# hamidthri/navbot_ppo

Measured on AMD Instinct MI355X. Metric: env_steps_per_sec, higher is better.
Workload: dtype f32; 1 GPU; BASELINE configs[1]: 4096 envs/GPU, stage_1 (32 segments), 10 beams, PPO mlp64x2, rollout=512, 50 full-batch epochs, episode cap 500; n_envs_total=4096, n_envs_per_gpu=4096, rollout_len=512, epochs=50, policy=mlp64x2, parallelism=env-shard dp1, update_arith=bf16x3, rollout=persistent kernel (navsim_rollout_mlp64)

## Files before the change

### navbot_ppo_amd/csrc/ppo_mlp64_x3s.h

```cpp
#pragma once

namespace x3s {

typedef unsigned u32x4 __attribute__((ext_vector_type(4)));
typedef unsigned u32x2 __attribute__((ext_vector_type(2)));
typedef short s16x4 __attribute__((ext_vector_type(4)));
typedef float v4f __attribute__((ext_vector_type(4)));

constexpr int SW = 4;
constexpr int kPieceB = 32 * 128;
constexpr int kImgB = 3 * kPieceB;

struct SmemS {
    uint16_t W2p[3][H][H];
    uint16_t W2Tp[3][H][H];
    uint16_t W1p[3][H][16];
    float b1[H], b2[H], w3[H], w4[H];
    unsigned char img[SW][2][kImgB];
};
static_assert(sizeof(SmemS) <= 160 * 1024, "LDS");
static_assert(offsetof(SmemS, img) % 128 == 0 && kImgB % 128 == 0, "image bases keep the low 7 address bits of a lane offset (the XOR swizzles)");
static_assert(sizeof(SmemS::img) >= 4 * ((Layout<16>::P_ACTOR + 6) & ~3) * sizeof(float), "reduction rows fit the images");
static_assert(sizeof(SmemS::img) / SW >= 96 * 64 * sizeof(float), "lane partials fit a wave's images");

#ifndef X3S_GUARD
#define X3S_GUARD ""
#endif
#define X3S_G "s_nop 0\n\t"
#define X3S_MFMA32_V_AV(acc, A, B) asm volatile(X3S_GUARD "v_mfma_f32_32x32x16_bf16 %0, %1, %2, %0" : "+v"(acc) : "a"(A), "v"(B))
#define X3S_MFMA32_V_AA(acc, A, B) asm volatile(X3S_GUARD "v_mfma_f32_32x32x16_bf16 %0, %1, %2, %0" : "+v"(acc) : "a"(A), "a"(B))
#define X3S_MFMA32G_V_AV(acc, A, B) asm volatile(X3S_G "v_mfma_f32_32x32x16_bf16 %0, %1, %2, %0" : "+v"(acc) : "a"(A), "v"(B))
#define X3S_MFMA32G_V_AA(acc, A, B) asm volatile(X3S_G "v_mfma_f32_32x32x16_bf16 %0, %1, %2, %0" : "+v"(acc) : "a"(A), "a"(B))
#define X3S_MFMA32_VZ_AV(acc, A, B) asm volatile(X3S_G "v_mfma_f32_32x32x16_bf16 %0, %1, %2, 0" : "=&v"(acc) : "a"(A), "v"(B))
#define X3S_MFMA32_VZ_AA(acc, A, B) asm volatile(X3S_G "v_mfma_f32_32x32x16_bf16 %0, %1, %2, 0" : "=&v"(acc) : "a"(A), "a"(B))
#define X3S_MFMA32_A_AV(acc, A, B) asm volatile(X3S_GUARD "v_mfma_f32_32x32x16_bf16 %0, %1, %2, %0" : "+a"(acc) : "a"(A), "v"(B))
#define X3S_MFMA32_AZ_AV(acc, A, B) asm volatile(X3S_G "v_mfma_f32_32x32x16_bf16 %0, %1, %2, 0" : "=&a"(acc) : "a"(A), "v"(B))
#define X3S_MFMA32_A_AA(acc, A, B) asm volatile(X3S_GUARD "v_mfma_f32_32x32x16_bf16 %0, %1, %2, %0" : "+a"(acc) : "a"(A), "a"(B))
#define X3S_MFMA16_A_AA(acc, A, B) asm volatile(X3S_GUARD "v_mfma_f32_16x16x32_bf16 %0, %1, %2, %0" : "+a"(acc) : "a"(A), "a"(B))
#define X3S_MFMA16G_A_AA(acc, A, B) asm volatile(X3S_G "v_mfma_f32_16x16x32_bf16 %0, %1, %2, %0" : "+a"(acc) : "a"(A), "a"(B))
#define X3S_MFMA16_A_AV(acc, A, B) asm volatile(X3S_GUARD "v_mfma_f32_16x16x32_bf16 %0, %1, %2, %0" : "+a"(acc) : "a"(A), "v"(B))

__device__ __forceinline__ void settle(f32x16& a, f32x16& b) { asm volatile("s_nop 7\n\ts_nop 3" : "+v"(a), "+v"(b)); }

__device__ __forceinline__ void split_a(unsigned& p0, float& ra, float& rb, const float a, const float b) {
    asm volatile("v_cvt_pk_bf16_f32 %0, %3, %4\n\t"
                 "v_lshlrev_b32 %1, 16, %0\n\t"
                 "v_and_b32 %2, 0xffff0000, %0\n\t"
                 "v_sub_f32 %1, %3, %1\n\t"
                 "v_sub_f32 %2, %4, %2"
                 : "=&v"(p0), "=&v"(ra), "=&v"(rb) : "v"(a), "v"(b));
}
__device__ __forceinline__ void split_b(unsigned& p1, unsigned& p2, const float ra, const float rb) {
    float t0, t1;
    asm volatile("v_cvt_pk_bf16_f32 %0, %4, %5\n\t"
                 "v_lshlrev_b32 %2, 16, %0\n\t"
                 "v_and_b32 %3, 0xffff0000, %0\n\t"
                 "v_sub_f32 %2, %4, %2\n\t"
                 "v_sub_f32 %3, %5, %3\n\t"
                 "v_cvt_pk_bf16_f32 %1, %2, %3"
                 : "=&v"(p1), "=&v"(p2), "=&v"(t0), "=&v"(t1) : "v"(ra), "v"(rb));
}
__device__ __forceinline__ void relu4(float (&h)[16], const f32x16& c, const int g) {
    float y0, y1, y2, y3;
    asm volatile("v_max_i32 %0, %4, 0\n\tv_max_i32 %1, %5, 0\n\tv_max_i32 %2, %6, 0\n\tv_max_i32 %3, %7, 0"
                 : "=&v"(y0), "=&v"(y1), "=&v"(y2), "=&v"(y3) : "v"(c[4 * g]), "v"(c[4 * g + 1]), "v"(c[4 * g + 2]), "v"(c[4 * g + 3]));
    h[4 * g] = y0; h[4 * g + 1] = y1; h[4 * g + 2] = y2; h[4 * g + 3] = y3;
}
template <bool ACTOR>
__device__ __forceinline__ void dh2_value(float& h, float& pw3, float& pw4, float& pb2, const float g3, const float g4, const float w3,
                                          const float w4) {
    float d;
    if constexpr (ACTOR)
        asm volatile("v_fmac_f32 %1, %0, %5\n\t"
                     "v_fmac_f32 %2, %0, %6\n\t"
                     "v_mul_f32 %4, %6, %8\n\t"
                     "v_fmac_f32 %4, %5, %7\n\t"
                     "v_cmp_lt_f32 vcc, 0, %0\n\t"
                     "v_cndmask_b32 %0, 0, %4, vcc\n\t"
                     "v_add_f32 %3, %3, %0"
                     : "+v"(h), "+v"(pw3), "+v"(pw4), "+v"(pb2), "=&v"(d) : "v"(g3), "v"(g4), "v"(w3), "v"(w4) : "vcc");
    else
        asm volatile("v_fmac_f32 %1, %0, %4\n\t"
                     "v_mul_f32 %3, %4, %5\n\t"
                     "v_cmp_lt_f32 vcc, 0, %0\n\t"
                     "v_cndmask_b32 %0, 0, %3, vcc\n\t"
                     "v_add_f32 %2, %2, %0"
                     : "+v"(h), "+v"(pw3), "+v"(pb2), "=&v"(d) : "v"(g3), "v"(w3) : "vcc");
}

__device__ __forceinline__ void mask4(float& y0, float& y1, float& y2, float& y3, const float x0, const float x1, const float x2,
                                      const float x3, const unsigned w0, const unsigned w1) {
    asm volatile("v_cmp_ne_u16 vcc, 0, %8\n\t"
                 "v_cndmask_b32 %0, 0, %4, vcc\n\t"
                 "v_cmp_lt_u32 vcc, 0xffff, %8\n\t"
                 "v_cndmask_b32 %1, 0, %5, vcc\n\t"
                 "v_cmp_ne_u16 vcc, 0, %9\n\t"
                 "v_cndmask_b32 %2, 0, %6, vcc\n\t"
                 "v_cmp_lt_u32 vcc, 0xffff, %9\n\t"
                 "v_cndmask_b32 %3, 0, %7, vcc"
                 : "=&v"(y0), "=&v"(y1), "=&v"(y2), "=&v"(y3) : "v"(x0), "v"(x1), "v"(x2), "v"(x3), "v"(w0), "v"(w1) : "vcc");
}

struct P3 {
    u32x4 p[3];
};

__device__ __forceinline__ int fswz(const int m) { return (m & 3) | ((((m >> 2) ^ (m >> 3)) & 1) << 2) | ((((m >> 1) ^ (m >> 3)) & 1) << 3); }

typedef __attribute__((address_space(3))) s16x4* lds_s16x4;
__device__ __forceinline__ u32x2 tr_read(const unsigned char* p) {
    const s16x4 v = __builtin_amdgcn_ds_read_tr16_b64_v4i16((lds_s16x4)p);
    u32x2 r;
    __builtin_memcpy(&r, &v, 8);
    return r;
}
__device__ __forceinline__ u32x4 cat(const u32x2 lo, const u32x2 hi) { return u32x4{lo.x, lo.y, hi.x, hi.y}; }

template <bool ACTOR>
__device__ __forceinline__ void pass_body(SmemS& sm, const float* __restrict__ params, const unsigned char* __restrict__ prep,
                                          const float* __restrict__ act, const float* __restrict__ logp_old,
                                          const float* __restrict__ rtg, const float* __restrict__ adv, long long M, float var,
                                          float clip, float inv_n, float* __restrict__ partial, float* __restrict__ stats_partial) {
    using L = Layout<16>;
    constexpr int OFF_W1 = L::OFF_W1, OFF_B1 = L::OFF_B1, OFF_W2 = L::OFF_W2, OFF_B2 = L::OFF_B2, OFF_W3 = L::OFF_W3, OFF_B3 = L::OFF_B3,
                  OFF_W4 = L::OFF_W4, OFF_B4 = L::OFF_B4;
    constexpr int P = ACTOR ? L::P_ACTOR : L::P_CRITIC;
    constexpr int NT = 64 * SW, kTileBytes = XPad<16>::kTileBytes, kRowsBytes = XPad<16>::kRowsBytes;
    const int tid = threadIdx.x, lane = tid & 63, wave = __builtin_amdgcn_readfirstlane(tid >> 6);
    const int l31 = lane & 31, lhi = lane >> 5, l15 = lane & 15, kk = lane >> 4;

    for (int k = tid; k < H * H / 2; k += NT) {
        const int r = (2 * k) / H, c = (2 * k) % H;
        uint32_t p0, p1, p2;
        bf16x3::split_pair(params[OFF_W2 + r * H + c], params[OFF_W2 + r * H + c + 1], p0, p1, p2);
        const uint32_t pc[3] = {p0, p1, p2};
#pragma unroll
        for (int i = 0; i < 3; ++i) {
            *reinterpret_cast<uint32_t*>(&sm.W2p[i][0][0] + wslot(r, kpos(c))) = pc[i];
            (&sm.W2Tp[i][0][0])[wslot(c, kpos(r))] = (uint16_t)(pc[i] & 0xffffu);
            (&sm.W2Tp[i][0][0])[wslot(c + 1, kpos(r))] = (uint16_t)(pc[i] >> 16);
        }
    }
    for (int k = tid; k < H * 16 / 2; k += NT) {
        const int r = (2 * k) / 16, c = (2 * k) % 16;
        uint32_t p0, p1, p2;
        bf16x3::split_pair(params[OFF_W1 + r * 16 + c], params[OFF_W1 + r * 16 + c + 1], p0, p1, p2);
        *reinterpret_cast<uint32_t*>(&sm.W1p[0][r][c]) = p0;
        *reinterpret_cast<uint32_t*>(&sm.W1p[1][r][c]) = p1;
        *reinterpret_cast<uint32_t*>(&sm.W1p[2][r][c]) = p2;
    }
    if (tid < H) {
        sm.b1[tid] = params[OFF_B1 + tid];
        sm.b2[tid] = params[OFF_B2 + tid];
        sm.w3[tid] = params[OFF_W3 + tid];
        sm.w4[tid] = ACTOR ? params[OFF_W4 + tid] : 0.f;
    }
    const float b3 = params[OFF_B3];
    const float b4 = ACTOR ? params[OFF_B4] : 0.f;
    __syncthreads();

    unsigned char* const smb = reinterpret_cast<unsigned char*>(&sm);
    const int img0 = (int)offsetof(SmemS, img) + wave * 2 * kImgB;
    constexpr int IMG_H = 0, IMG_D = kImgB;
    const int st_base = img0 + l31 * 128 + ((fswz(l31) ^ lhi) << 3);
    auto st_off = [&](const int t, const int j, const int b) { return st_base ^ ((8 * t + 4 * j + 2 * b) << 3); };
    const int g_row = 8 * lhi + (l15 >> 2), g_quad = 4 * ((lane >> 4) & 1) + (lane & 3);
    const int g_base0 = img0 + g_row * 128 + ((g_quad ^ fswz(g_row)) << 3), g_base1 = img0 + (g_row + 4) * 128 + ((g_quad ^ fswz(g_row + 4)) << 3);
    auto g_off = [&](const int t, const int s, const int rd) { return ((rd ? g_base1 : g_base0) ^ (t << 6)) + s * 2048; };
    const int h_row = 8 * kk + (l15 >> 2), h_quad = lane & 3;
    const int h_base0 = img0 + h_row * 128 + ((h_quad ^ fswz(h_row)) << 3), h_base1 = img0 + (h_row + 4) * 128 + ((h_quad ^ fswz(h_row + 4)) << 3);
    auto ldw = [&](const uint16_t* base, const int tt, const int s, const int i) {
        return *reinterpret_cast<const u32x4*>(base + i * H * H + wslot(32 * tt + l31, 16 * s + 8 * lhi));
    };
    const int vec_off = 4 * lhi;
    auto ldv = [&](const float* v, const int t, const int g) { return *reinterpret_cast<const v4f*>(v + 32 * t + 8 * g + vec_off); };

    f32x16 aW2[2][2];
    v4f aW1[4], aB1[4];
#pragma unroll
    for (int a = 0; a < 2; ++a)
#pragma unroll
        for (int b = 0; b < 2; ++b) aW2[a][b] = zero16();
#pragma unroll
    for (int u = 0; u < 4; ++u) aW1[u] = aB1[u] = v4f{0.f, 0.f, 0.f, 0.f};
    float pb2[2][16], pw3[2][16], pw4[2][16];
#pragma unroll
    for (int t = 0; t < 2; ++t)
#pragma unroll
        for (int r = 0; r < 16; ++r) pb2[t][r] = pw3[t][r] = pw4[t][r] = 0.f;
    float adb3 = 0.f, adb4 = 0.f, st0 = 0.f, st1 = 0.f, st2 = 0.f, st3 = 0.f;
    u32x4 ones = {0x3f803f80u, 0x3f803f80u, 0x3f803f80u, 0x3f803f80u};
    asm volatile("" : "+a"(ones));

    const long long n_tiles = (M + 31) / 32;
    const long long gw = (long long)blockIdx.x * SW + wave, stride = (long long)gridDim.x * SW;
    u32x4 xp[3], xbn[3];
    float pre_a0 = 0.f, pre_a1 = 0.f, pre_lp = 0.f, pre_t = 0.f;
    auto request_tile = [&](const long long next, const long long cur) {
        const unsigned char* r = prep + (size_t)next * kTileBytes + ((l31 * 3) * 16 + 8 * lhi) * 2;
        const unsigned char* c = prep + (size_t)cur * kTileBytes + kRowsBytes + (l15 * 32 + 8 * kk) * 2;
        asm volatile("global_load_dwordx4 %0, %3, off\n\tglobal_load_dwordx4 %1, %3, off offset:32\n\tglobal_load_dwordx4 %2, %3, off offset:64"
                     : "=a"(xp[0]), "=a"(xp[1]), "=a"(xp[2]) : "v"(r));
        asm volatile("global_load_dwordx4 %0, %3, off\n\tglobal_load_dwordx4 %1, %3, off offset:1024\n\tglobal_load_dwordx4 %2, %3, off offset:2048"
                     : "=a"(xbn[0]), "=a"(xbn[1]), "=a"(xbn[2]) : "v"(c));
        const long long m = next * 32 + l31;
        if (m < M) {
            if (ACTOR) {
                const float2 a = reinterpret_cast<const float2*>(act)[m];
                pre_a0 = a.x;
                pre_a1 = a.y;
                pre_lp = logp_old[m];
                pre_t = adv[m];
            } else {
                pre_t = rtg[m];
            }
        }
    };
    auto landed = [&]() {
        asm volatile("s_waitcnt vmcnt(0)" : "+a"(xp[0]), "+a"(xp[1]), "+a"(xp[2]), "+a"(xbn[0]), "+a"(xbn[1]), "+a"(xbn[2]));
    };
    static_assert(kTileBytes == 6144 && kRowsBytes == 3072, "offsets of the asm loads: pieces 32 bytes apart in a row, 1024 in the columns");

    struct G1Ops {
        P3 da[4];
    };
    auto g1_gather_pair = [&](G1Ops& o, const int q, const int hb0, const int hb1) {
        const int u = q / 3, i = q % 3;
        o.da[u].p[i] = cat(tr_read(smb + (hb0 ^ (u << 5)) + IMG_D + i * kPieceB), tr_read(smb + (hb1 ^ (u << 5)) + IMG_D + i * kPieceB));
    };
    auto g1_step = [&](const int k, const G1Ops& o, const u32x4 (&xb)[3], const bool guard = false) {
        const int t1 = k / 18, q = k % 18, u = 2 * t1 + (q & 1), e = q >> 1;
        constexpr int kind[9] = {0, 1, 0, 0, 1, 0, 0, 1, 0};
        constexpr int ai[9] = {2, 2, 1, 0, 1, 1, 0, 0, 0};
        constexpr int bi[9] = {0, 0, 1, 2, 0, 0, 1, 0, 0};
        if (guard) {
            if (kind[e]) { X3S_MFMA16G_A_AA(aB1[u], o.da[u].p[ai[e]], ones); }
            else { X3S_MFMA16G_A_AA(aW1[u], o.da[u].p[ai[e]], xb[bi[e]]); }
        } else {
            if (kind[e]) { X3S_MFMA16_A_AA(aB1[u], o.da[u].p[ai[e]], ones); }
            else { X3S_MFMA16_A_AA(aW1[u], o.da[u].p[ai[e]], xb[bi[e]]); }
        }
    };
    auto store_pieces = [&](const int img, const int t, const int j, const P3& q) {
#pragma unroll
        for (int i = 0; i < 3; ++i) {
            *reinterpret_cast<u32x2*>(smb + st_off(t, j, 0) + img + i * kPieceB) = u32x2{q.p[i].x, q.p[i].y};
            *reinterpret_cast<u32x2*>(smb + st_off(t, j, 1) + img + i * kPieceB) = u32x2{q.p[i].z, q.p[i].w};
        }
    };
    struct SplitState {
        float ra[4], rb[4];
    };
    auto split_block = [&](const float (&c)[16], const int j, const int b, P3& q, SplitState& ss) {
        const int pr = b >> 1;
        if ((b & 1) == 0) {
            unsigned p0;
            split_a(p0, ss.ra[pr], ss.rb[pr], c[8 * j + 2 * pr], c[8 * j + 2 * pr + 1]);
            q.p[0][pr] = p0;
        } else {
            unsigned p1, p2;
            split_b(p1, p2, ss.ra[pr], ss.rb[pr]);
            q.p[1][pr] = p1;
            q.p[2][pr] = p2;
        }
    };

    for (int k = lane; k < kImgB / 16; k += 64) reinterpret_cast<u32x4*>(smb + img0 + IMG_D)[k] = u32x4{0u, 0u, 0u, 0u};
    bool have_prev = false;
    if (gw < n_tiles) {
        request_tile(gw, gw);
        landed();
    }
    for (long long tile = gw; tile < n_tiles; tile += stride) {
        const bool valid = tile * 32 + l31 < M;
        const u32x4 xr[3] = {xp[0], xp[1], xp[2]}, xb[3] = {xbn[0], xbn[1], xbn[2]};
        const float cur_a0 = pre_a0, cur_a1 = pre_a1, cur_lp = pre_lp, cur_t = pre_t;

        f32x16 c1[2];
#pragma unroll
        for (int q = 0; q < 8; ++q) {
            const v4f b = ldv(sm.b1, q >> 2, q & 3);
            c1[q >> 2][4 * (q & 3)] = b.x; c1[q >> 2][4 * (q & 3) + 1] = b.y; c1[q >> 2][4 * (q & 3) + 2] = b.z; c1[q >> 2][4 * (q & 3) + 3] = b.w;
        }
        {
            u32x4 wa[2][3];
#pragma unroll
            for (int t = 0; t < 2; ++t)
#pragma unroll
                for (int i = 0; i < 3; ++i) wa[t][i] = *reinterpret_cast<const u32x4*>(&sm.W1p[i][32 * t + l31][8 * lhi]);
            X3S_MFMA32G_V_AA(c1[0], wa[0][2], xr[0]); X3S_MFMA32G_V_AA(c1[1], wa[1][2], xr[0]);
            X3S_MFMA32_V_AA(c1[0], wa[0][1], xr[1]);  X3S_MFMA32_V_AA(c1[1], wa[1][1], xr[1]);
            X3S_MFMA32_V_AA(c1[0], wa[0][0], xr[2]);  X3S_MFMA32_V_AA(c1[1], wa[1][0], xr[2]);
            X3S_MFMA32_V_AA(c1[0], wa[0][1], xr[0]);  X3S_MFMA32_V_AA(c1[1], wa[1][1], xr[0]);
            X3S_MFMA32_V_AA(c1[0], wa[0][0], xr[1]);  X3S_MFMA32_V_AA(c1[1], wa[1][0], xr[1]);
            X3S_MFMA32_V_AA(c1[0], wa[0][0], xr[0]);  X3S_MFMA32_V_AA(c1[1], wa[1][0], xr[0]);
        }
        request_tile(tile + stride < n_tiles ? tile + stride : tile, tile);
        u32x4 wn[2][3];
#pragma unroll
        for (int i = 0; i < 3; ++i) {
            wn[0][i] = ldw(&sm.W2p[0][0][0], 0, 0, i);
            wn[1][i] = ldw(&sm.W2p[0][0][0], 1, 0, i);
        }
        settle(c1[0], c1[1]);
        float h1[2][16];
#pragma unroll
        for (int q = 0; q < 8; ++q) relu4(h1[q >> 2], c1[q >> 2], q & 3);
        f32x16 c2[2];
#pragma unroll
        for (int q = 0; q < 8; ++q) {
            const v4f b = ldv(sm.b2, q >> 2, q & 3);
            c2[q >> 2][4 * (q & 3)] = b.x; c2[q >> 2][4 * (q & 3) + 1] = b.y; c2[q >> 2][4 * (q & 3) + 2] = b.z; c2[q >> 2][4 * (q & 3) + 3] = b.w;
        }

        G1Ops g1o;
        {
            P3 hb[4];
            u32x4 wk[4][2];
            SplitState ss;
#pragma unroll
            for (int b = 0; b < 8; ++b) split_block(h1[0], 0, b, hb[0], ss);
#pragma unroll
            for (int s = 0; s < 4; ++s) {
                u32x4 w[2][3];
#pragma unroll
                for (int i = 0; i < 3; ++i) { w[0][i] = wn[0][i]; w[1][i] = wn[1][i]; }
                auto filler = [&](const int slot) {
                    if (s < 3 && slot >= 1 && slot <= 8) split_block(h1[(s + 1) >> 1], (s + 1) & 1, slot - 1, hb[s + 1], ss);
                    if (s == 3 && slot < 8) wk[slot >> 1][slot & 1] = ldw(&sm.W2p[0][0][0], slot & 1, slot >> 1, 0);
                    if (s < 3 && (slot == 0 || slot == 4 || slot == 9)) {
                        const int i = slot == 0 ? 0 : slot == 4 ? 1 : 2;
                        wn[0][i] = ldw(&sm.W2p[0][0][0], 0, s + 1, i);
                        wn[1][i] = ldw(&sm.W2p[0][0][0], 1, s + 1, i);
                    }
                    if (slot == 9) store_pieces(IMG_H, s >> 1, s & 1, hb[s]);
                };
                if (s == 0) { X3S_MFMA32G_V_AV(c2[0], w[0][2], hb[s].p[0]); } else { X3S_MFMA32_V_AV(c2[0], w[0][2], hb[s].p[0]); }
                filler(0);
                if (s == 0) { X3S_MFMA32G_V_AV(c2[1], w[1][2], hb[s].p[0]); } else { X3S_MFMA32_V_AV(c2[1], w[1][2], hb[s].p[0]); }
                filler(1);
                X3S_MFMA32_V_AV(c2[0], w[0][1], hb[s].p[1]); filler(2);
                X3S_MFMA32_V_AV(c2[1], w[1][1], hb[s].p[1]); filler(3);
                X3S_MFMA32_V_AV(c2[0], w[0][0], hb[s].p[2]); filler(4);
                X3S_MFMA32_V_AV(c2[1], w[1][0], hb[s].p[2]); filler(5);
                X3S_MFMA32_V_AV(c2[0], w[0][1], hb[s].p[0]); filler(6);
                X3S_MFMA32_V_AV(c2[1], w[1][1], hb[s].p[0]); filler(7);
                X3S_MFMA32_V_AV(c2[0], w[0][0], hb[s].p[1]); filler(8);
                X3S_MFMA32_V_AV(c2[1], w[1][0], hb[s].p[1]); filler(9);
            }
            int hb0 = h_base0, hb1 = h_base1;
            asm volatile("" : "+v"(hb0), "+v"(hb1));
            int gq = 0;
#pragma unroll
            for (int s = 0; s < 4; ++s) {
                X3S_MFMA32_V_AV(c2[0], wk[s][0], hb[s].p[0]);
                g1_gather_pair(g1o, gq++, hb0, hb1); g1_gather_pair(g1o, gq++, hb0, hb1);
                X3S_MFMA32_V_AV(c2[1], wk[s][1], hb[s].p[0]);
                g1_gather_pair(g1o, gq++, hb0, hb1);
            }
        }
        settle(c2[0], c2[1]);

        int g1k = 0;
        float h2[2][16];
#pragma unroll
        for (int q = 0; q < 8; ++q) {
            relu4(h2[q >> 2], c2[q >> 2], q & 3);
            g1_step(g1k++, g1o, xb);
            g1_step(g1k++, g1o, xb);
        }
        float g3 = 0.f, g4 = 0.f;
        {
            float z3 = 0.f, z4 = 0.f;
#pragma unroll
            for (int t = 0; t < 2; ++t)
#pragma unroll
                for (int g = 0; g < 4; ++g) {
                    const v4f w = ldv(sm.w3, t, g);
                    z3 = fmaf(h2[t][4 * g], w.x, z3); z3 = fmaf(h2[t][4 * g + 1], w.y, z3);
                    z3 = fmaf(h2[t][4 * g + 2], w.z, z3); z3 = fmaf(h2[t][4 * g + 3], w.w, z3);
                    if (ACTOR) {
                        const v4f v = ldv(sm.w4, t, g);
                        z4 = fmaf(h2[t][4 * g], v.x, z4); z4 = fmaf(h2[t][4 * g + 1], v.y, z4);
                        z4 = fmaf(h2[t][4 * g + 2], v.z, z4); z4 = fmaf(h2[t][4 * g + 3], v.w, z4);
                    }
                }
            z3 += __shfl_xor(z3, 32, 64);
            if (ACTOR) z4 += __shfl_xor(z4, 32, 64);
            const float own = (lhi == 0) ? 1.f : 0.f;
            if (valid) {
                z3 += b3;
                z4 += b4;
#ifdef MLP64_DEBUG_Z
                if (lhi == 0) {
                    float* const dbg = partial + (size_t)200 * P;
                    dbg[tile * 32 + l31] = z3;
                    if (ACTOR) dbg[M + tile * 32 + l31] = z4;
                }
#endif
                if (ACTOR) {
                    const float mu0 = 1.0f / (1.0f + expf(-z3));
                    const float mu1 = tanhf(z4);
                    const float d0 = cur_a0 - mu0, d1 = cur_a1 - mu1;
                    const float lp = -0.5f * ((d0 * d0 + d1 * d1) / var) - 1.8378770664093453f - logf(var);
                    const float lr = lp - cur_lp;
                    const float ratio = expf(lr);
                    const float A = cur_t;
                    const float s1 = ratio * A;
                    const float rc = fminf(fmaxf(ratio, 1.0f - clip), 1.0f + clip);
                    const float s2 = rc * A;
                    st0 += own * -fminf(s1, s2);
                    st2 += own * ((ratio - 1.0f) - lr);
                    st3 += (fabsf(ratio - 1.0f) > clip) ? own : 0.f;
                    const bool inside = (ratio >= 1.0f - clip) && (ratio <= 1.0f + clip);
                    const float dL_dratio = (inside || s1 < s2) ? -A : 0.f;
                    const float dL_dlp = dL_dratio * ratio * inv_n;
                    g3 = dL_dlp * (d0 / var) * (mu0 * (1.0f - mu0));
                    g4 = dL_dlp * (d1 / var) * (1.0f - mu1 * mu1);
                } else {
                    const float e = z3 - cur_t;
                    st1 += own * (e * e);
                    g3 = 2.0f * e * inv_n;
                }
            }
            adb3 += own * g3;
            adb4 += own * g4;
#ifdef MLP64_DEBUG_Z
            if (valid && lhi == 0) {
                float* const dbg = partial + (size_t)200 * P;
                dbg[2 * M + tile * 32 + l31] = g3;
                if (ACTOR) dbg[3 * M + tile * 32 + l31] = g4;
            }
#endif
        }
        {
            v4f wn3 = ldv(sm.w3, 0, 0), wn4 = ACTOR ? ldv(sm.w4, 0, 0) : v4f{0.f, 0.f, 0.f, 0.f};
#pragma unroll
            for (int q = 0; q < 8; ++q) {
                const int t = q >> 2, g = q & 3;
                const v4f w = wn3, v = wn4;
                if (q < 7) {
                    wn3 = ldv(sm.w3, (q + 1) >> 2, (q + 1) & 3);
                    if (ACTOR) wn4 = ldv(sm.w4, (q + 1) >> 2, (q + 1) & 3);
                }
                const float wv3[4] = {w.x, w.y, w.z, w.w}, wv4[4] = {v.x, v.y, v.z, v.w};
#pragma unroll
                for (int j = 0; j < 4; ++j) {
                    const int r = 4 * g + j;
                    dh2_value<ACTOR>(h2[t][r], pw3[t][r], pw4[t][r], pb2[t][r], g3, g4, wv3[j], wv4[j]);
                    if (g1k < 36 && (j & 1)) g1_step(g1k++, g1o, xb);
                }
                if (g1k < 36 && (g & 1)) g1_step(g1k++, g1o, xb);
            }
        }
        while (g1k < 36) g1_step(g1k++, g1o, xb);

        f32x16 c3[2];
        P3 hB[2][2], dA[2][2];
        u32x2 mw[8];
        {
            P3 db[4];
            u32x4 wk[4][2];
            SplitState ss;
#pragma unroll
            for (int i = 0; i < 3; ++i) {
                wn[0][i] = ldw(&sm.W2Tp[0][0][0], 0, 0, i);
                wn[1][i] = ldw(&sm.W2Tp[0][0][0], 1, 0, i);
            }
#pragma unroll
            for (int b = 0; b < 8; ++b) split_block(h2[0], 0, b, db[0], ss);
#pragma unroll
            for (int s = 0; s < 4; ++s) {
                u32x4 w[2][3];
#pragma unroll
                for (int i = 0; i < 3; ++i) { w[0][i] = wn[0][i]; w[1][i] = wn[1][i]; }
                auto filler = [&](const int slot) {
                    if (s < 3 && slot >= 1 && slot <= 8) split_block(h2[(s + 1) >> 1], (s + 1) & 1, slot - 1, db[s + 1], ss);
                    if (s == 3 && slot < 8) wk[slot >> 1][slot & 1] = ldw(&sm.W2Tp[0][0][0], slot & 1, slot >> 1, 0);
                    if (slot == 2 || slot == 5 || slot == 8) {
                        const int q = 3 * s + (slot - 2) / 3, t = q / 6, sk = (q / 3) & 1, i = q % 3;
                        hB[t][sk].p[i] = cat(tr_read(smb + g_off(t, sk, 0) + IMG_H + i * kPieceB), tr_read(smb + g_off(t, sk, 1) + IMG_H + i * kPieceB));
                    }
                    if (s == 3 && (slot == 3 || slot == 4 || slot == 6 || slot == 7)) {
                        const int k0 = 2 * (slot - 3 - (slot > 4));
#pragma unroll
                        for (int k = k0; k < k0 + 2; ++k)
                            mw[k] = *reinterpret_cast<const u32x2*>(smb + st_off(k >> 2, (k >> 1) & 1, k & 1) + IMG_H);
                    }
                    if (s < 3 && (slot == 0 || slot == 4 || slot == 9)) {
                        const int i = slot == 0 ? 0 : slot == 4 ? 1 : 2;
                        wn[0][i] = ldw(&sm.W2Tp[0][0][0], 0, s + 1, i);
                        wn[1][i] = ldw(&sm.W2Tp[0][0][0], 1, s + 1, i);
                    }
                    if (slot == 9) store_pieces(IMG_D, s >> 1, s & 1, db[s]);
                };
                if (s == 0) { X3S_MFMA32_VZ_AV(c3[0], w[0][2], db[s].p[0]); } else { X3S_MFMA32_V_AV(c3[0], w[0][2], db[s].p[0]); }
                filler(0);
                if (s == 0) { X3S_MFMA32_VZ_AV(c3[1], w[1][2], db[s].p[0]); } else { X3S_MFMA32_V_AV(c3[1], w[1][2], db[s].p[0]); }
                filler(1);
                X3S_MFMA32_V_AV(c3[0], w[0][1], db[s].p[1]); filler(2);
                X3S_MFMA32_V_AV(c3[1], w[1][1], db[s].p[1]); filler(3);
                X3S_MFMA32_V_AV(c3[0], w[0][0], db[s].p[2]); filler(4);
                X3S_MFMA32_V_AV(c3[1], w[1][0], db[s].p[2]); filler(5);
                X3S_MFMA32_V_AV(c3[0], w[0][1], db[s].p[0]); filler(6);
                X3S_MFMA32_V_AV(c3[1], w[1][1], db[s].p[0]); filler(7);
                X3S_MFMA32_V_AV(c3[0], w[0][0], db[s].p[1]); filler(8);
                X3S_MFMA32_V_AV(c3[1], w[1][0], db[s].p[1]); filler(9);
            }
            int dq = 0;
            auto gather_d = [&]() {
                const int t = dq / 6, sk = (dq / 3) & 1, i = dq % 3;
                dA[t][sk].p[i] = cat(tr_read(smb + g_off(t, sk, 0) + IMG_D + i * kPieceB), tr_read(smb + g_off(t, sk, 1) + IMG_D + i * kPieceB));
                ++dq;
            };
#pragma unroll
            for (int s = 0; s < 4; ++s) {
                X3S_MFMA32_V_AV(c3[0], wk[s][0], db[s].p[0]);
                gather_d(); gather_d();
                X3S_MFMA32_V_AV(c3[1], wk[s][1], db[s].p[0]);
                gather_d();
            }
        }

        {
            settle(c3[0], c3[1]);
            float d1[2][16];
#pragma unroll
            for (int k = 0; k < 8; ++k) {
                const int t = k >> 2, r0 = 8 * ((k >> 1) & 1) + 4 * (k & 1);
                mask4(d1[t][r0], d1[t][r0 + 1], d1[t][r0 + 2], d1[t][r0 + 3], c3[t][r0], c3[t][r0 + 1], c3[t][r0 + 2], c3[t][r0 + 3], mw[k].x, mw[k].y);
            }
            P3 eb[4];
            SplitState ss;
            int blk = 0;
            auto filler = [&]() {
                if (blk < 32) {
                    const int s = blk >> 3;
                    split_block(d1[s >> 1], s & 1, blk & 7, eb[s], ss);
                    if ((blk & 7) == 7) store_pieces(IMG_D, s >> 1, s & 1, eb[s]);
                }
                ++blk;
            };
#pragma unroll
            for (int t2 = 0; t2 < 2; ++t2)
#pragma unroll
                for (int s = 0; s < 2; ++s) {
                    const P3& A = dA[t2][s];
                    const P3 &B0 = hB[0][s], &B1 = hB[1][s];
                    f32x16 &a0 = aW2[t2][0], &a1 = aW2[t2][1];
                    X3S_MFMA32_A_AA(a0, A.p[2], B0.p[0]); filler(); X3S_MFMA32_A_AA(a1, A.p[2], B1.p[0]); filler();
                    X3S_MFMA32_A_AA(a0, A.p[1], B0.p[1]); filler(); X3S_MFMA32_A_AA(a1, A.p[1], B1.p[1]); filler();
                    X3S_MFMA32_A_AA(a0, A.p[0], B0.p[2]); filler(); X3S_MFMA32_A_AA(a1, A.p[0], B1.p[2]); filler();
                    X3S_MFMA32_A_AA(a0, A.p[1], B0.p[0]); filler(); X3S_MFMA32_A_AA(a1, A.p[1], B1.p[0]); filler();
                    X3S_MFMA32_A_AA(a0, A.p[0], B0.p[1]); filler(); X3S_MFMA32_A_AA(a1, A.p[0], B1.p[1]); filler();
                    X3S_MFMA32_A_AA(a0, A.p[0], B0.p[0]); filler(); X3S_MFMA32_A_AA(a1, A.p[0], B1.p[0]); filler();
                }
        }
        landed();
        have_prev = true;
    }
    if (have_prev) {
        const u32x4 xb[3] = {xbn[0], xbn[1], xbn[2]};
        G1Ops g1o;
#pragma unroll
        for (int q = 0; q < 12; ++q) g1_gather_pair(g1o, q, h_base0, h_base1);
#pragma unroll
        for (int k = 0; k < 36; ++k) g1_step(k, g1o, xb, true);
    }

    __syncthreads();
    float rb2[2], rw3[2], rw4[2];
    {
        float* const scr = reinterpret_cast<float*>(&sm.img[wave][0][0]);
#pragma unroll
        for (int t = 0; t < 2; ++t)
#pragma unroll
            for (int r = 0; r < 16; ++r) {
                scr[(0 * 32 + 16 * t + r) * 64 + lane] = pb2[t][r];
                scr[(1 * 32 + 16 * t + r) * 64 + lane] = pw3[t][r];
                scr[(2 * 32 + 16 * t + r) * 64 + lane] = pw4[t][r];
            }
        __builtin_amdgcn_fence(__ATOMIC_RELEASE, "wavefront");
        __builtin_amdgcn_wave_barrier();
        const int row = l31, hi = (row >> 2) & 1, r = (row & 3) + 4 * (row >> 3), t = lhi;
        float s[3] = {0.f, 0.f, 0.f};
#pragma unroll
        for (int v = 0; v < 3; ++v) {
            const float* src = scr + (v * 32 + 16 * t + r) * 64 + 32 * hi;
#pragma unroll
            for (int m = 0; m < 32; m += 4) {
                const v4f q = *reinterpret_cast<const v4f*>(src + m);
                s[v] += (q.x + q.y) + (q.z + q.w);
            }
        }
        rb2[0] = s[0]; rw3[0] = s[1]; rw4[0] = s[2];
        rb2[1] = rw3[1] = rw4[1] = 0.f;
    }
    __syncthreads();

    constexpr int RP = (P + 3 + 3) & ~3;
    float s3 = adb3, s4 = adb4, sA = ACTOR ? st0 : st1, sB = st2, sC = st3;
#pragma unroll
    for (int o = 32; o >= 1; o >>= 1) {
        s3 += __shfl_xor(s3, o, 64); s4 += __shfl_xor(s4, o, 64);
        sA += __shfl_xor(sA, o, 64); sB += __shfl_xor(sB, o, 64); sC += __shfl_xor(sC, o, 64);
    }
    float* const red0 = reinterpret_cast<float*>(&sm.img[0][0][0]);
    float* const rowp = red0 + wave * RP;
    {
        auto put = [&](int idx, float v) { rowp[idx] = v; };
#pragma unroll
        for (int t2 = 0; t2 < 2; ++t2)
#pragma unroll
            for (int t1 = 0; t1 < 2; ++t1)
#pragma unroll
                for (int r = 0; r < 16; ++r) put(OFF_W2 + (32 * t2 + c_row(r, lane)) * H + 32 * t1 + l31, aW2[t2][t1][r]);
        put(OFF_B2 + 32 * lhi + l31, rb2[0]);
        put(OFF_W3 + 32 * lhi + l31, rw3[0]);
        if (ACTOR) put(OFF_W4 + 32 * lhi + l31, rw4[0]);
#pragma unroll
        for (int u = 0; u < 4; ++u) {
#pragma unroll
            for (int r = 0; r < 4; ++r) put(OFF_W1 + (16 * u + 4 * kk + r) * 16 + l15, aW1[u][r]);
            if (l15 == 0) {
#pragma unroll
                for (int r = 0; r < 4; ++r) put(OFF_B1 + 16 * u + 4 * kk + r, aB1[u][r]);
            }
        }
        if (lane == 0) {
            put(OFF_B3, s3);
            if (ACTOR) put(OFF_B4, s4);
            put(P + 0, sA);
            put(P + 1, sB);
            put(P + 2, sC);
        }
    }
    __syncthreads();
    float* out = partial + (size_t)blockIdx.x * P;
    const float* red = red0;
    for (int k = tid; k < P; k += NT) out[k] = (red[k] + red[RP + k]) + (red[2 * RP + k] + red[3 * RP + k]);
    if (tid < 3) stats_partial[blockIdx.x * 4 + tid] = (red[P + tid] + red[RP + P + tid]) + (red[2 * RP + P + tid] + red[3 * RP + P + tid]);
}

}

__global__ __launch_bounds__(64 * x3s::SW) void mlp64_pass_both_x3s(const float* __restrict__ params, const unsigned char* __restrict__ prep,
                                                                    const float* __restrict__ act, const float* __restrict__ logp_old,
                                                                    const float* __restrict__ rtg, const float* __restrict__ adv,
                                                                    long long M, float var, float clip, float inv_n, int net_mask,
                                                                    float* __restrict__ partial_a, float* __restrict__ stats_partial_a,
                                                                    float* __restrict__ partial_c, float* __restrict__ stats_partial_c) {
    __shared__ __attribute__((aligned(128))) x3s::SmemS sm;
    if (net_mask & 1) x3s::pass_body<true>(sm, params, prep, act, logp_old, rtg, adv, M, var, clip, inv_n, partial_a, stats_partial_a);
    if (net_mask == 3) __syncthreads();
    if (net_mask & 2) x3s::pass_body<false>(sm, params + Layout<16>::P_ACTOR, prep, act, logp_old, rtg, adv, M, var, clip, inv_n, partial_c, stats_partial_c);
}
```

Measured before the change: 52.91 million env-steps/s.

## Software-pipeline next tile's layer-1 forward into the W2 gradient MFMA stream

Restructures the PPO update loop so the next tile's first-layer forward MFMAs, bias loads, ReLU and split work are interleaved into the slot schedule of the current tile's W2-gradient MFMAs. The tile load is split into separate row, column and scalar requests issued at different points, so the global loads overlap compute. The d-mask and error splitting are spread across the same slots, and some bias-gradient accumulators move to VGPRs to balance register files. This aims to hide MFMA dependency stalls and load latency, but adds register pressure and tight hand-scheduled ordering that can spill or mis-order the asm loads.

```diff
diff --git a/navbot_ppo_amd/csrc/ppo_mlp64_x3s.h b/navbot_ppo_amd/csrc/ppo_mlp64_x3s.h
--- a/navbot_ppo_amd/csrc/ppo_mlp64_x3s.h
+++ b/navbot_ppo_amd/csrc/ppo_mlp64_x3s.h
@@ -37,8 +37,14 @@
 #define X3S_MFMA32_AZ_AV(acc, A, B) asm volatile(X3S_G "v_mfma_f32_32x32x16_bf16 %0, %1, %2, 0" : "=&a"(acc) : "a"(A), "v"(B))
 #define X3S_MFMA32_A_AA(acc, A, B) asm volatile(X3S_GUARD "v_mfma_f32_32x32x16_bf16 %0, %1, %2, %0" : "+a"(acc) : "a"(A), "a"(B))
 #define X3S_MFMA16_A_AA(acc, A, B) asm volatile(X3S_GUARD "v_mfma_f32_16x16x32_bf16 %0, %1, %2, %0" : "+a"(acc) : "a"(A), "a"(B))
+#define X3S_MFMA16_V_AA(acc, A, B) asm volatile(X3S_GUARD "v_mfma_f32_16x16x32_bf16 %0, %1, %2, %0" : "+v"(acc) : "a"(A), "a"(B))
+#define X3S_MFMA16G_V_AA(acc, A, B) asm volatile(X3S_G "v_mfma_f32_16x16x32_bf16 %0, %1, %2, %0" : "+v"(acc) : "a"(A), "a"(B))
+#define X3S_MFMA16_A_VA(acc, A, B) asm volatile(X3S_GUARD "v_mfma_f32_16x16x32_bf16 %0, %1, %2, %0" : "+a"(acc) : "v"(A), "a"(B))
+#define X3S_MFMA16_V_VA(acc, A, B) asm volatile(X3S_GUARD "v_mfma_f32_16x16x32_bf16 %0, %1, %2, %0" : "+v"(acc) : "v"(A), "a"(B))
 #define X3S_MFMA16G_A_AA(acc, A, B) asm volatile(X3S_G "v_mfma_f32_16x16x32_bf16 %0, %1, %2, %0" : "+a"(acc) : "a"(A), "a"(B))
 #define X3S_MFMA16_A_AV(acc, A, B) asm volatile(X3S_GUARD "v_mfma_f32_16x16x32_bf16 %0, %1, %2, %0" : "+a"(acc) : "a"(A), "v"(B))
+
+#define X3S_REP10(F, b) F(b + 0); F(b + 1); F(b + 2); F(b + 3); F(b + 4); F(b + 5); F(b + 6); F(b + 7); F(b + 8); F(b + 9);
 
 __device__ __forceinline__ void settle(f32x16& a, f32x16& b) { asm volatile("s_nop 7\n\ts_nop 3" : "+v"(a), "+v"(b)); }
 
@@ -189,6 +195,7 @@
 #pragma unroll
         for (int r = 0; r < 16; ++r) pb2[t][r] = pw3[t][r] = pw4[t][r] = 0.f;
     float adb3 = 0.f, adb4 = 0.f, st0 = 0.f, st1 = 0.f, st2 = 0.f, st3 = 0.f;
+    auto keep_w2 = [&]() { asm volatile("" : "+a"(aW2[0][0]), "+a"(aW2[0][1]), "+a"(aW2[1][0]), "+a"(aW2[1][1])); };
     u32x4 ones = {0x3f803f80u, 0x3f803f80u, 0x3f803f80u, 0x3f803f80u};
     asm volatile("" : "+a"(ones));
 
@@ -196,14 +203,18 @@
     const long long gw = (long long)blockIdx.x * SW + wave, stride = (long long)gridDim.x * SW;
     u32x4 xp[3], xbn[3];
     float pre_a0 = 0.f, pre_a1 = 0.f, pre_lp = 0.f, pre_t = 0.f;
-    auto request_tile = [&](const long long next, const long long cur) {
-        const unsigned char* r = prep + (size_t)next * kTileBytes + ((l31 * 3) * 16 + 8 * lhi) * 2;
-        const unsigned char* c = prep + (size_t)cur * kTileBytes + kRowsBytes + (l15 * 32 + 8 * kk) * 2;
+    auto request_rows = [&](const long long t) {
+        const unsigned char* r = prep + (size_t)t * kTileBytes + ((l31 * 3) * 16 + 8 * lhi) * 2;
         asm volatile("global_load_dwordx4 %0, %3, off\n\tglobal_load_dwordx4 %1, %3, off offset:32\n\tglobal_load_dwordx4 %2, %3, off offset:64"
                      : "=a"(xp[0]), "=a"(xp[1]), "=a"(xp[2]) : "v"(r));
+    };
+    auto request_cols = [&](const long long t) {
+        const unsigned char* c = prep + (size_t)t * kTileBytes + kRowsBytes + (l15 * 32 + 8 * kk) * 2;
         asm volatile("global_load_dwordx4 %0, %3, off\n\tglobal_load_dwordx4 %1, %3, off offset:1024\n\tglobal_load_dwordx4 %2, %3, off offset:2048"
                      : "=a"(xbn[0]), "=a"(xbn[1]), "=a"(xbn[2]) : "v"(c));
-        const long long m = next * 32 + l31;
+    };
+    auto request_scalars = [&](const long long t) {
+        const long long m = t * 32 + l31;
         if (m < M) {
             if (ACTOR) {
                 const float2 a = reinterpret_cast<const float2*>(act)[m];
@@ -234,11 +245,16 @@
         constexpr int ai[9] = {2, 2, 1, 0, 1, 1, 0, 0, 0};
         constexpr int bi[9] = {0, 0, 1, 2, 0, 0, 1, 0, 0};
         if (guard) {
-            if (kind[e]) { X3S_MFMA16G_A_AA(aB1[u], o.da[u].p[ai[e]], ones); }
+            if (kind[e]) { X3S_MFMA16G_V_AA(aB1[u], o.da[u].p[ai[e]], ones); }
             else { X3S_MFMA16G_A_AA(aW1[u], o.da[u].p[ai[e]], xb[bi[e]]); }
         } else {
-            if (kind[e]) { X3S_MFMA16_A_AA(aB1[u], o.da[u].p[ai[e]], ones); }
-            else { X3S_MFMA16_A_AA(aW1[u], o.da[u].p[ai[e]], xb[bi[e]]); }
+            if (ACTOR) {
+                if (kind[e]) { X3S_MFMA16_V_AA(aB1[u], o.da[u].p[ai[e]], ones); }
+                else { X3S_MFMA16_A_AA(aW1[u], o.da[u].p[ai[e]], xb[bi[e]]); }
+            } else {
+                if (kind[e]) { X3S_MFMA16_V_VA(aB1[u], o.da[u].p[ai[e]], ones); }
+                else { X3S_MFMA16_A_VA(aW1[u], o.da[u].p[ai[e]], xb[bi[e]]); }
+            }
         }
     };
     auto store_pieces = [&](const int img, const int t, const int j, const P3& q) {
@@ -265,66 +281,77 @@
         }
     };
 
+    f32x16 c1[2], c2[2];
+    float h1[2][16];
+    P3 hb[4];
+    u32x4 wn[2][3], wa[2][3];
+    SplitState ss1;
+    auto g2_step = [&](const int k, const P3 (&dA)[2][2], const P3 (&hB)[2][2], f32x16 (&aW2)[2][2]) {
+        const int t2 = k / 24, sk = (k / 12) & 1, e = (k % 12) >> 1, t1 = k & 1;
+        constexpr int ai[6] = {2, 1, 0, 1, 0, 0}, bi[6] = {0, 1, 2, 0, 1, 0};
+        X3S_MFMA32_A_AA(aW2[t2][t1], dA[t2][sk].p[ai[e]], hB[t1][sk].p[bi[e]]);
+    };
+    auto b1_to_c1 = [&](const int q) {
+        const v4f b = ldv(sm.b1, q >> 2, q & 3);
+        c1[q >> 2][4 * (q & 3)] = b.x; c1[q >> 2][4 * (q & 3) + 1] = b.y; c1[q >> 2][4 * (q & 3) + 2] = b.z; c1[q >> 2][4 * (q & 3) + 3] = b.w;
+    };
+    auto b2_to_c2 = [&](const int q) {
+        const v4f b = ldv(sm.b2, q >> 2, q & 3);
+        c2[q >> 2][4 * (q & 3)] = b.x; c2[q >> 2][4 * (q & 3) + 1] = b.y; c2[q >> 2][4 * (q & 3) + 2] = b.z; c2[q >> 2][4 * (q & 3) + 3] = b.w;
+    };
+    auto ld_wa = [&](const int t, const int i) { wa[t][i] = *reinterpret_cast<const u32x4*>(&sm.W1p[i][32 * t + l31][8 * lhi]); };
+    auto ld_wn = [&](const int t, const int i) { wn[t][i] = ldw(&sm.W2p[0][0][0], t, 0, i); };
+    auto f1_mfma = [&](const int j) {
+        const int t = j / 6, e = j % 6;
+        constexpr int wi[6] = {2, 1, 0, 1, 0, 0}, xi[6] = {0, 1, 2, 0, 1, 0};
+        if (e == 0) { X3S_MFMA32G_V_AA(c1[t], wa[t][wi[e]], xp[xi[e]]); } else { X3S_MFMA32_V_AA(c1[t], wa[t][wi[e]], xp[xi[e]]); }
+    };
+    auto ahead_work = [&](const int n, const bool alone) {
+        if (n == 11 || n == 13) ld_wa(0, (n - 11) / 2);
+        if (n == 15 || n == 17) ld_wa(1, (n - 15) / 2);
+        if (n == 19) { ld_wa(0, 2); ld_wa(1, 2); }
+        if (n >= 22 && n <= 29) b1_to_c1(n - 22);
+        if (n == 42) { ld_wn(0, 0); ld_wn(1, 0); ld_wn(0, 1); ld_wn(1, 1); }
+        if (n == 43) {
+            ld_wn(0, 2); ld_wn(1, 2);
+            if (alone) asm volatile("s_nop 7" : "+v"(c1[0]));
+            relu4(h1[0], c1[0], 0);
+        }
+        if (n == 44) relu4(h1[0], c1[0], 1);
+        if (n >= 45 && n <= 52) { split_block(h1[0], 0, n - 45, hb[0], ss1); b2_to_c2(n - 45); }
+        if (n == 53) relu4(h1[0], c1[0], 2);
+        if (n == 54) relu4(h1[0], c1[0], 3);
+        if (n >= 55 && n <= 58) relu4(h1[1], c1[1], n - 55);
+    };
+
     for (int k = lane; k < kImgB / 16; k += 64) reinterpret_cast<u32x4*>(smb + img0 + IMG_D)[k] = u32x4{0u, 0u, 0u, 0u};
     bool have_prev = false;
     if (gw < n_tiles) {
-        request_tile(gw, gw);
-        landed();
+        request_rows(gw);
+        request_cols(gw);
+        request_scalars(gw);
+        auto slot = [&](const int n) {
+            if (n == 36) landed();
+            if (n >= 36 && n < 48) f1_mfma(n - 36);
+            ahead_work(n, true);
+        };
+        X3S_REP10(slot, 10) X3S_REP10(slot, 20) X3S_REP10(slot, 30) X3S_REP10(slot, 40) X3S_REP10(slot, 50)
     }
     for (long long tile = gw; tile < n_tiles; tile += stride) {
         const bool valid = tile * 32 + l31 < M;
-        const u32x4 xr[3] = {xp[0], xp[1], xp[2]}, xb[3] = {xbn[0], xbn[1], xbn[2]};
         const float cur_a0 = pre_a0, cur_a1 = pre_a1, cur_lp = pre_lp, cur_t = pre_t;
-
-        f32x16 c1[2];
-#pragma unroll
-        for (int q = 0; q < 8; ++q) {
-            const v4f b = ldv(sm.b1, q >> 2, q & 3);
-            c1[q >> 2][4 * (q & 3)] = b.x; c1[q >> 2][4 * (q & 3) + 1] = b.y; c1[q >> 2][4 * (q & 3) + 2] = b.z; c1[q >> 2][4 * (q & 3) + 3] = b.w;
-        }
-        {
-            u32x4 wa[2][3];
-#pragma unroll
-            for (int t = 0; t < 2; ++t)
-#pragma unroll
-                for (int i = 0; i < 3; ++i) wa[t][i] = *reinterpret_cast<const u32x4*>(&sm.W1p[i][32 * t + l31][8 * lhi]);
-            X3S_MFMA32G_V_AA(c1[0], wa[0][2], xr[0]); X3S_MFMA32G_V_AA(c1[1], wa[1][2], xr[0]);
-            X3S_MFMA32_V_AA(c1[0], wa[0][1], xr[1]);  X3S_MFMA32_V_AA(c1[1], wa[1][1], xr[1]);
-            X3S_MFMA32_V_AA(c1[0], wa[0][0], xr[2]);  X3S_MFMA32_V_AA(c1[1], wa[1][0], xr[2]);
-            X3S_MFMA32_V_AA(c1[0], wa[0][1], xr[0]);  X3S_MFMA32_V_AA(c1[1], wa[1][1], xr[0]);
-            X3S_MFMA32_V_AA(c1[0], wa[0][0], xr[1]);  X3S_MFMA32_V_AA(c1[1], wa[1][0], xr[1]);
-            X3S_MFMA32_V_AA(c1[0], wa[0][0], xr[0]);  X3S_MFMA32_V_AA(c1[1], wa[1][0], xr[0]);
-        }
-        request_tile(tile + stride < n_tiles ? tile + stride : tile, tile);
-        u32x4 wn[2][3];
-#pragma unroll
-        for (int i = 0; i < 3; ++i) {
-            wn[0][i] = ldw(&sm.W2p[0][0][0], 0, 0, i);
-            wn[1][i] = ldw(&sm.W2p[0][0][0], 1, 0, i);
-        }
-        settle(c1[0], c1[1]);
-        float h1[2][16];
-#pragma unroll
-        for (int q = 0; q < 8; ++q) relu4(h1[q >> 2], c1[q >> 2], q & 3);
-        f32x16 c2[2];
-#pragma unroll
-        for (int q = 0; q < 8; ++q) {
-            const v4f b = ldv(sm.b2, q >> 2, q & 3);
-            c2[q >> 2][4 * (q & 3)] = b.x; c2[q >> 2][4 * (q & 3) + 1] = b.y; c2[q >> 2][4 * (q & 3) + 2] = b.z; c2[q >> 2][4 * (q & 3) + 3] = b.w;
-        }
+        const long long tile1 = tile + stride < n_tiles ? tile + stride : tile;
 
         G1Ops g1o;
         {
-            P3 hb[4];
             u32x4 wk[4][2];
             SplitState ss;
 #pragma unroll
-            for (int b = 0; b < 8; ++b) split_block(h1[0], 0, b, hb[0], ss);
-#pragma unroll
             for (int s = 0; s < 4; ++s) {
                 u32x4 w[2][3];
 #pragma unroll
                 for (int i = 0; i < 3; ++i) { w[0][i] = wn[0][i]; w[1][i] = wn[1][i]; }
+                keep_w2();
                 auto filler = [&](const int slot) {
                     if (s < 3 && slot >= 1 && slot <= 8) split_block(h1[(s + 1) >> 1], (s + 1) & 1, slot - 1, hb[s + 1], ss);
                     if (s == 3 && slot < 8) wk[slot >> 1][slot & 1] = ldw(&sm.W2p[0][0][0], slot & 1, slot >> 1, 0);
@@ -362,12 +389,12 @@
         settle(c2[0], c2[1]);
 
         int g1k = 0;
+        keep_w2();
         float h2[2][16];
 #pragma unroll
         for (int q = 0; q < 8; ++q) {
+            g1_step(g1k++, g1o, xbn);
             relu4(h2[q >> 2], c2[q >> 2], q & 3);
-            g1_step(g1k++, g1o, xb);
-            g1_step(g1k++, g1o, xb);
         }
         float g3 = 0.f, g4 = 0.f;
         {
@@ -448,33 +475,44 @@
                 for (int j = 0; j < 4; ++j) {
                     const int r = 4 * g + j;
                     dh2_value<ACTOR>(h2[t][r], pw3[t][r], pw4[t][r], pb2[t][r], g3, g4, wv3[j], wv4[j]);
-                    if (g1k < 36 && (j & 1)) g1_step(g1k++, g1o, xb);
+                    if (g1k < 36 && (j & 1)) g1_step(g1k++, g1o, xbn);
                 }
-                if (g1k < 36 && (g & 1)) g1_step(g1k++, g1o, xb);
-            }
-        }
-        while (g1k < 36) g1_step(g1k++, g1o, xb);
+                if (g1k < 36 && (g & 1)) g1_step(g1k++, g1o, xbn);
+            }
+        }
 
         f32x16 c3[2];
         P3 hB[2][2], dA[2][2];
         u32x2 mw[8];
+        float d1[2][16];
+        auto d_mask = [&](const int k) {
+            const int t = k >> 2, r0 = 8 * ((k >> 1) & 1) + 4 * (k & 1);
+            mask4(d1[t][r0], d1[t][r0 + 1], d1[t][r0 + 2], d1[t][r0 + 3], c3[t][r0], c3[t][r0 + 1], c3[t][r0 + 2], c3[t][r0 + 3], mw[k].x, mw[k].y);
+        };
         {
             P3 db[4];
-            u32x4 wk[4][2];
+            u32x4 wk[4][2], wt[2][3];
             SplitState ss;
 #pragma unroll
             for (int i = 0; i < 3; ++i) {
-                wn[0][i] = ldw(&sm.W2Tp[0][0][0], 0, 0, i);
-                wn[1][i] = ldw(&sm.W2Tp[0][0][0], 1, 0, i);
-            }
-#pragma unroll
-            for (int b = 0; b < 8; ++b) split_block(h2[0], 0, b, db[0], ss);
+                wt[0][i] = ldw(&sm.W2Tp[0][0][0], 0, 0, i);
+                wt[1][i] = ldw(&sm.W2Tp[0][0][0], 1, 0, i);
+            }
+#pragma unroll
+            for (int b = 0; b < 8; ++b) {
+                g1_step(g1k++, g1o, xbn);
+                split_block(h2[0], 0, b, db[0], ss);
+            }
 #pragma unroll
             for (int s = 0; s < 4; ++s) {
                 u32x4 w[2][3];
 #pragma unroll
-                for (int i = 0; i < 3; ++i) { w[0][i] = wn[0][i]; w[1][i] = wn[1][i]; }
+                for (int i = 0; i < 3; ++i) { w[0][i] = wt[0][i]; w[1][i] = wt[1][i]; }
+                keep_w2();
                 auto filler = [&](const int slot) {
+                    if (s == 0 && slot == 0) request_cols(tile);
+                    if (s == 0 && slot == 1) request_rows(tile1);
+                    if (s == 3 && slot == 0) request_scalars(tile1);
                     if (s < 3 && slot >= 1 && slot <= 8) split_block(h2[(s + 1) >> 1], (s + 1) & 1, slot - 1, db[s + 1], ss);
                     if (s == 3 && slot < 8) wk[slot >> 1][slot & 1] = ldw(&sm.W2Tp[0][0][0], slot & 1, slot >> 1, 0);
                     if (slot == 2 || slot == 5 || slot == 8) {
@@ -489,8 +527,8 @@
                     }
                     if (s < 3 && (slot == 0 || slot == 4 || slot == 9)) {
                         const int i = slot == 0 ? 0 : slot == 4 ? 1 : 2;
-                        wn[0][i] = ldw(&sm.W2Tp[0][0][0], 0, s + 1, i);
-                        wn[1][i] = ldw(&sm.W2Tp[0][0][0], 1, s + 1, i);
+                        wt[0][i] = ldw(&sm.W2Tp[0][0][0], 0, s + 1, i);
+                        wt[1][i] = ldw(&sm.W2Tp[0][0][0], 1, s + 1, i);
                     }
                     if (slot == 9) store_pieces(IMG_D, s >> 1, s & 1, db[s]);
                 };
@@ -517,55 +555,44 @@
             for (int s = 0; s < 4; ++s) {
                 X3S_MFMA32_V_AV(c3[0], wk[s][0], db[s].p[0]);
                 gather_d(); gather_d();
+            }
+#pragma unroll
+            for (int s = 0; s < 4; ++s) {
                 X3S_MFMA32_V_AV(c3[1], wk[s][1], db[s].p[0]);
-                gather_d();
+                if (s < 2) { gather_d(); gather_d(); }
+                else d_mask(s - 2);
             }
         }
 
         {
-            settle(c3[0], c3[1]);
-            float d1[2][16];
-#pragma unroll
-            for (int k = 0; k < 8; ++k) {
-                const int t = k >> 2, r0 = 8 * ((k >> 1) & 1) + 4 * (k & 1);
-                mask4(d1[t][r0], d1[t][r0 + 1], d1[t][r0 + 2], d1[t][r0 + 3], c3[t][r0], c3[t][r0 + 1], c3[t][r0 + 2], c3[t][r0 + 3], mw[k].x, mw[k].y);
-            }
             P3 eb[4];
             SplitState ss;
-            int blk = 0;
-            auto filler = [&]() {
-                if (blk < 32) {
-                    const int s = blk >> 3;
-                    split_block(d1[s >> 1], s & 1, blk & 7, eb[s], ss);
-                    if ((blk & 7) == 7) store_pieces(IMG_D, s >> 1, s & 1, eb[s]);
-                }
-                ++blk;
+            auto d_work = [&](const int n) {
+                if (n == 0 || n == 1) d_mask(2 + n);
+                if (n == 20 || n == 21) d_mask(4 + n - 20);
+                if (n == 31 || n == 32) d_mask(6 + n - 31);
+                const int s = n < 11 ? 0 : n < 20 ? 1 : n < 31 ? 2 : 3, n0 = s == 0 ? 2 : s == 1 ? 11 : s == 2 ? 22 : 33;
+                if (n >= n0 && n < n0 + 8) split_block(d1[s >> 1], s & 1, n - n0, eb[s], ss);
+                if (n == n0 + 8) store_pieces(IMG_D, s >> 1, s & 1, eb[s]);
             };
-#pragma unroll
-            for (int t2 = 0; t2 < 2; ++t2)
-#pragma unroll
-                for (int s = 0; s < 2; ++s) {
-                    const P3& A = dA[t2][s];
-                    const P3 &B0 = hB[0][s], &B1 = hB[1][s];
-                    f32x16 &a0 = aW2[t2][0], &a1 = aW2[t2][1];
-                    X3S_MFMA32_A_AA(a0, A.p[2], B0.p[0]); filler(); X3S_MFMA32_A_AA(a1, A.p[2], B1.p[0]); filler();
-                    X3S_MFMA32_A_AA(a0, A.p[1], B0.p[1]); filler(); X3S_MFMA32_A_AA(a1, A.p[1], B1.p[1]); filler();
-                    X3S_MFMA32_A_AA(a0, A.p[0], B0.p[2]); filler(); X3S_MFMA32_A_AA(a1, A.p[0], B1.p[2]); filler();
-                    X3S_MFMA32_A_AA(a0, A.p[1], B0.p[0]); filler(); X3S_MFMA32_A_AA(a1, A.p[1], B1.p[0]); filler();
-                    X3S_MFMA32_A_AA(a0, A.p[0], B0.p[1]); filler(); X3S_MFMA32_A_AA(a1, A.p[0], B1.p[1]); filler();
-                    X3S_MFMA32_A_AA(a0, A.p[0], B0.p[0]); filler(); X3S_MFMA32_A_AA(a1, A.p[0], B1.p[0]); filler();
-                }
-        }
-        landed();
+            auto slot = [&](const int n) {
+                if (n == 36) landed();
+                if (n < 36) g2_step(n, dA, hB, aW2);
+                else if (n < 48) f1_mfma(n - 36);
+                else g2_step(n - 12, dA, hB, aW2);
+                d_work(n);
+                ahead_work(n, false);
+            };
+            X3S_REP10(slot, 0) X3S_REP10(slot, 10) X3S_REP10(slot, 20) X3S_REP10(slot, 30) X3S_REP10(slot, 40) X3S_REP10(slot, 50)
+        }
         have_prev = true;
     }
     if (have_prev) {
-        const u32x4 xb[3] = {xbn[0], xbn[1], xbn[2]};
         G1Ops g1o;
 #pragma unroll
         for (int q = 0; q < 12; ++q) g1_gather_pair(g1o, q, h_base0, h_base1);
 #pragma unroll
-        for (int k = 0; k < 36; ++k) g1_step(k, g1o, xb, true);
+        for (int k = 0; k < 36; ++k) g1_step(k, g1o, xbn, true);
     }
 
     __syncthreads();
```

New measurement: 55.28 million env-steps/s, median of 6. 4.5% higher.
